# Guenael/rtlsdr-wsprd

Hardware: AMD Instinct MI355X
Metric: 2-minute WSPR segments decoded per second (higher is better)
Workload: dtype f32

## Files before the change

### rtlsdr-wsprd_amd/csrc/kernels/fano_wave.h

```cpp
#pragma once
#include <stdint.h>

#if defined(__HIPCC__)
#define WSPR_FW_HD __host__ __device__ __forceinline__
#else
#define WSPR_FW_HD static inline
#endif

namespace wspr {
namespace fano_wave {

constexpr int kBits = 81, kLast = 80, kTail = 81 - 31, kDelta = 60;
constexpr uint32_t kPolyA = 0xf2d05351u, kPolyB = 0xe4613c47u;
constexpr int kPosDone = 127;

struct Visit { uint32_t st, dlo, meta, gt, led; };

WSPR_FW_HD int      v_pos(const Visit& v)   { return (int)((v.meta >> 18) & 127u); }
WSPR_FW_HD bool     v_retry(const Visit& v) { return (v.meta >> 25) & 1u; }
WSPR_FW_HD int      v_gamma(const Visit& v) { return (int)(int16_t)(v.gt & 0xffffu); }
WSPR_FW_HD int      v_thr(const Visit& v)   { return (int)(int16_t)(v.gt >> 16); }
WSPR_FW_HD uint32_t pack_gt(int g, int t)   { return ((uint32_t)g & 0xffffu) | ((uint32_t)t << 16); }
WSPR_FW_HD uint32_t pack_meta(uint32_t dhi, int pos, bool retry) {
    return (dhi & 0x3ffffu) | ((uint32_t)pos << 18) | ((uint32_t)retry << 25);
}

WSPR_FW_HD unsigned parity32(uint32_t v) {
#if defined(__HIP_DEVICE_COMPILE__)
    return (unsigned)__popc(v) & 1u;
#else
    return (unsigned)__builtin_popcount(v) & 1u;
#endif
}

struct Expansion {
    bool has0, has1, again, done;
    uint32_t look1;
    Visit kid0, kid1, self;
};

WSPR_FW_HD int metric_of(uint32_t lo, uint32_t hi, unsigned pair) {
    const uint32_t w = (pair & 2u) ? hi : lo;
    return (int)(int16_t)((pair & 1u) ? (w >> 16) : (w & 0xffffu));
}

WSPR_FW_HD void expand(const Visit& v, uint32_t bm_lo, uint32_t bm_hi, Expansion& e) {
    const int pos = v_pos(v), g = v_gamma(v), t = v_thr(v);
    const bool tail = pos >= kTail;
    const unsigned zp = (parity32(v.st & kPolyA) << 1) | parity32(v.st & kPolyB);
    const int m0 = metric_of(bm_lo, bm_hi, zp), m1 = metric_of(bm_lo, bm_hi, 3u ^ zp);
    const bool zero_better = tail || (m0 > m1);
    const int best = zero_better ? m0 : m1, second = zero_better ? m1 : m0;
    const uint32_t better = zero_better ? 0u : 1u;
    const int a0 = g + best, a1 = g + second;
    const bool first_visit = g < t + kDelta;
    const bool ok0 = a0 >= t;
    const bool ok1 = ok0 && !tail && a1 >= t;
    e.done = ok0 && pos == kLast;
    e.has0 = ok0 && !e.done;
    e.has1 = ok1;
    e.look1 = (ok0 && !tail) ? 1u : 0u;
    e.again = v_retry(v) && !e.done;
    const bool up0 = first_visit && a0 >= t + kDelta;
    const bool up1 = first_visit && a1 >= t + kDelta;
    uint32_t dlo0 = v.dlo, dhi0 = v.meta & 0x3ffffu, dlo1 = v.dlo, dhi1 = dhi0;
    if (pos < 32)      { dlo0 |= better << pos;        dlo1 |= (better ^ 1u) << pos; }
    else if (pos < 50) { dhi0 |= better << (pos - 32); dhi1 |= (better ^ 1u) << (pos - 32); }
    e.kid0.st = (v.st | better) << 1;
    e.kid0.dlo = dlo0;
    e.kid0.meta = pack_meta(dhi0, pos + 1, up0);
    e.kid0.gt = pack_gt(a0, up0 ? t + kDelta : t);
    e.kid0.led = 0;
    e.kid1.st = (v.st | (better ^ 1u)) << 1;
    e.kid1.dlo = dlo1;
    e.kid1.meta = pack_meta(dhi1, pos + 1, up1);
    e.kid1.gt = pack_gt(a1, up1 ? t + kDelta : t);
    e.kid1.led = 0;
    e.self = v;
    e.self.meta = pack_meta(v.meta & 0x3ffffu, pos, pos == 0);
    e.self.gt = pack_gt(g, t - kDelta);
    e.self.led = 0;
    if (e.done) {
        e.self = v;
        e.self.meta = pack_meta(v.meta & 0x3ffffu, kPosDone, false);
        e.self.gt = pack_gt(a0, t);
    }
}

WSPR_FW_HD void decisions_to_bytes(uint32_t dlo, uint32_t dhi, unsigned char* data10) {
    for (int k = 0; k < 10; ++k) {
        unsigned b = 0;
        for (int j = 0; j < 8; ++j) {
            const int n = 8 * k + j;
            const unsigned bit = n < 32 ? (dlo >> n) & 1u : (n < 50 ? (dhi >> (n - 32)) & 1u : 0u);
            b = (b << 1) | bit;
        }
        data10[k] = (unsigned char)b;
    }
}

struct Result {
    int ret;
    unsigned cycles;
    unsigned metric;
    unsigned steps;
    unsigned char data[10];
};

}
}
```

### rtlsdr-wsprd_amd/csrc/kernels/k6_fano_wave.hip

```cpp
#include "wspr_device.h"
#include "fano_wave.h"
#include <cstdlib>
#include <algorithm>

namespace wspr {
namespace {

using namespace fano_wave;


__device__ __forceinline__ uint32_t wave_scan_add(uint32_t v) {
#define WSPR_DPP(x, ctrl, rmask, bmask) (uint32_t)__builtin_amdgcn_update_dpp(0, (int)(x), ctrl, rmask, bmask, false)
    v += WSPR_DPP(v, 0x111, 0xf, 0xf);
    v += WSPR_DPP(v, 0x112, 0xf, 0xf);
    v += WSPR_DPP(v, 0x114, 0xf, 0xe);
    v += WSPR_DPP(v, 0x118, 0xf, 0xc);
    v += WSPR_DPP(v, 0x142, 0xa, 0xf);
    v += WSPR_DPP(v, 0x143, 0xc, 0xf);
#undef WSPR_DPP
    return v;
}

__device__ __forceinline__ int lanes_below(unsigned long long mask) {
    return (int)__builtin_amdgcn_mbcnt_hi((unsigned)(mask >> 32), __builtin_amdgcn_mbcnt_lo((unsigned)mask, 0u));
}

constexpr int kWin = 512, kHalf = kWin / 2;
static_assert(kHalf >= 64 && kWin - 192 >= kHalf, "a step's pops (<= 64) and pushes (<= 192) must fit beside the half that moves");

template <int kCap>
__global__ __launch_bounds__(64)
void fano_wave_kernel(const unsigned char* __restrict__ symbols, const int* __restrict__ offsets, int n,
                      const short* __restrict__ metric0, unsigned maxcycles,
                      int* __restrict__ ret, unsigned* __restrict__ cycles, unsigned* __restrict__ metric,
                      unsigned* __restrict__ maxnp, unsigned char* __restrict__ data, unsigned* __restrict__ steps_out,
                      uint32_t* __restrict__ gpool, int* __restrict__ next_vector) {
    __shared__ uint32_t lpool[5 * kWin];
    uint32_t* __restrict__ gp = gpool + (size_t)blockIdx.x * 5 * kCap;
    auto ld = [&](int arr, int i) -> uint32_t { return lpool[arr * kWin + (i & (kWin - 1))]; };
    auto st_ = [&](int arr, int i, uint32_t v) { lpool[arr * kWin + (i & (kWin - 1))] = v; };
    auto lds_order = [] {
        __builtin_amdgcn_fence(__ATOMIC_RELEASE, "wavefront");
        __builtin_amdgcn_wave_barrier();
        __builtin_amdgcn_fence(__ATOMIC_ACQUIRE, "wavefront");
    };
    __shared__ uint2 bm[kBits];
    __shared__ unsigned char symd[kNSymD];
    __shared__ short mt[256];
    const int lane = threadIdx.x;
    for (int e = lane; e < 256; e += 64) mt[e] = metric0[e];
    for (;;) {
    int v;
    if (next_vector) {
        int got = 0;
        if (lane == 0) got = atomicAdd(next_vector, 1);
        v = __builtin_amdgcn_readfirstlane(got);
    } else {
        v = blockIdx.x;
    }
    if (v >= n) return;
    __syncthreads();

    {
        const unsigned char* __restrict__ sym = symbols + (size_t)offsets[v] * kNSymD;
        int base = 0;
        for (int c = 0; c < 4; ++c) {
            const int i = 64 * c + lane;
            const int j = (int)(__brev((unsigned)i) >> 24);
            const bool valid = j < kNSymD;
            const unsigned long long m = __ballot(valid);
            if (valid) symd[base + lanes_below(m)] = sym[j];
            base += __popcll(m);
        }
    }
    __syncthreads();
    for (int k = lane; k < kBits; k += 64) {
        const int s0 = symd[2 * k], s1 = symd[2 * k + 1];
        const int a0 = mt[s0], a1 = mt[255 - s0], b0 = mt[s1], b1 = mt[255 - s1];
        bm[k] = make_uint2((uint32_t)(uint16_t)(short)(a0 + b0) | ((uint32_t)(uint16_t)(short)(a0 + b1) << 16),
                           (uint32_t)(uint16_t)(short)(a1 + b0) | ((uint32_t)(uint16_t)(short)(a1 + b1) << 16));
    }
    if (lane == 0) {
        st_(0, 0, 0u); st_(1, 0, 0u); st_(2, 0, pack_meta(0u, 0, true)); st_(3, 0, pack_gt(0, 0)); st_(4, 0, 0u);
    }
    __syncthreads();

    const unsigned budget = maxcycles * (unsigned)kBits;
    int size = 1;
    int lo = 0;
    unsigned settled = 0;
    unsigned steps = 0;
    int rc = -2;
    unsigned out_cycles = 0, out_metric = 0;
    uint32_t out_dlo = 0, out_dhi = 0;

    for (;;) {
        if (settled >= budget) { rc = -1; out_cycles = budget + 2; break; }
        const int room = kCap - size;
        const int wide = size <= kCap / 2 ? 64 : (room > 256 ? 8 : 1);
        const int take = min(min(wide, size), room >> 1);
        if (take < 1 || steps > 4u * budget + 1024u) { rc = -2; break; }
        ++steps;
        if (size - take < lo) {
            __builtin_amdgcn_fence(__ATOMIC_RELEASE, "workgroup");
            __builtin_amdgcn_fence(__ATOMIC_ACQUIRE, "workgroup");
            lo -= kHalf;
#pragma unroll
            for (int arr = 0; arr < 5; ++arr)
#pragma unroll
                for (int u = 0; u < kHalf / 64; ++u) {
                    const int i = lo + 64 * u + lane;
                    lpool[arr * kWin + (i & (kWin - 1))] = gp[arr * kCap + i];
                }
            lds_order();
        }
        const bool active = lane < take;
        const int idx = size - 1 - (active ? lane : 0);
        Visit x{ld(0, idx), ld(1, idx), ld(2, idx), ld(3, idx), ld(4, idx)};
        const int pos = v_pos(x);
        const bool is_done_visit = active && pos == kPosDone;
        if (__builtin_amdgcn_readfirstlane((int)is_done_visit)) {
            const unsigned looks = settled + 1;
            rc = looks >= budget ? -1 : 0;
            out_cycles = looks + 1;
            out_metric = (unsigned)__builtin_amdgcn_readfirstlane(v_gamma(x));
            out_dlo = (uint32_t)__builtin_amdgcn_readfirstlane((int)x.dlo);
            out_dhi = (uint32_t)__builtin_amdgcn_readfirstlane((int)(x.meta & 0x3ffffu));
            break;
        }
        const uint2 q = bm[min(pos, kLast)];
        Expansion e;
        expand(x, q.x, q.y, e);
        const bool stop_here = active && (is_done_visit || e.done);
        const unsigned long long stop_mask = __ballot(stop_here);
        bool live = active;
        int base = size - take;
        if (stop_mask) {
            const int jc = __builtin_ctzll(stop_mask);
            live = active && lane <= jc;
            base = 0;
            lo = 0;
        }
        const bool keep_self = live && (is_done_visit || e.done);
        const bool has0 = live && !keep_self && e.has0;
        const bool has1 = live && !keep_self && e.has1;
        const bool again = live && (keep_self || e.again);
        const int c = (int)has0 + (int)has1 + (int)again;
        if (__ballot(again && !keep_self && v_thr(e.self) < -32000)) { rc = -2; break; }
        const unsigned long long b0 = __ballot(has0), b1 = __ballot(has1), b2 = __ballot(again);
        const int before = lanes_below(b0) + lanes_below(b1) + lanes_below(b2);
        const int total = __popcll(b0) + __popcll(b1) + __popcll(b2);
        const uint32_t back = (live && !keep_self) ? 1u + (c == 0 ? x.led : 0u) : 0u;
        const uint32_t pre = wave_scan_add(back);
        const unsigned long long has_mask = b0 | b1 | b2;
        const unsigned long long later = has_mask & ~((2ull << lane) - 1ull);
        const int nxt = later ? __builtin_ctzll(later) : 63;
        const uint32_t pre_nxt = (uint32_t)__builtin_amdgcn_ds_bpermute(nxt << 2, (int)pre);
        const uint32_t gain = pre_nxt - pre;
        const int first = has_mask ? __builtin_ctzll(has_mask) : 63;
        settled += (uint32_t)__builtin_amdgcn_readlane((int)pre, first);
        if (base + total > lo + kWin) {
#pragma unroll
            for (int arr = 0; arr < 5; ++arr)
#pragma unroll
                for (int u = 0; u < kHalf / 64; ++u) {
                    const int i = lo + 64 * u + lane;
                    gp[arr * kCap + i] = lpool[arr * kWin + (i & (kWin - 1))];
                }
            lo += kHalf;
            lds_order();
        }
        const int top = base + total - 1;
        const uint32_t tail_led = x.led + gain;
        if (has0) {
            const int w = top - before;
            st_(0, w, e.kid0.st); st_(1, w, e.kid0.dlo); st_(2, w, e.kid0.meta); st_(3, w, e.kid0.gt);
            st_(4, w, e.look1 + ((!has1 && !again) ? tail_led : 0u));
        }
        if (has1) {
            const int w = top - before - (int)has0;
            st_(0, w, e.kid1.st); st_(1, w, e.kid1.dlo); st_(2, w, e.kid1.meta); st_(3, w, e.kid1.gt);
            st_(4, w, !again ? tail_led : 0u);
        }
        if (again) {
            const int w = top - before - (int)has0 - (int)has1;
            const Visit s = is_done_visit ? x : e.self;
            st_(0, w, s.st); st_(1, w, s.dlo); st_(2, w, s.meta); st_(3, w, s.gt);
            st_(4, w, keep_self ? 0u : tail_led);
        }
        size = base + total;
        lds_order();
    }
    if (lane == 0) {
        ret[v] = rc;
        cycles[v] = out_cycles;
        if (metric) metric[v] = rc == 0 ? out_metric : 0u;
        if (maxnp) maxnp[v] = rc == 0 ? (unsigned)kLast : 0u;
        unsigned char d[10];
        decisions_to_bytes(out_dlo, out_dhi, d);
        for (int k = 0; k < 10; ++k) data[(size_t)v * 10 + k] = d[k];
        if (steps_out) steps_out[v] = steps;
    }
    if (!next_vector) return;
    }
}

}

#ifndef WSPR_K6W_PER_CU
#define WSPR_K6W_PER_CU 13
#endif
constexpr int kWaveGrid = 256 * WSPR_K6W_PER_CU;

size_t fano_wave_scratch_words(int n) {
    return (size_t)std::min(n, kWaveGrid) * 5 * 4096 + 16;
}

void launch_fano_wave(const unsigned char* symbols, const int* offsets, int n, const short* metric0,
                      unsigned maxcycles, int* ret, unsigned* cycles, unsigned* metric, unsigned* maxnp,
                      unsigned char* data, unsigned* steps, uint32_t* scratch, hipStream_t st) {
    if (n <= 0) return;
    const int grid = std::min(n, kWaveGrid);
    int* counter = reinterpret_cast<int*>(scratch + (size_t)grid * 5 * 4096);
    static const int rep = [] { const char* e = lab_env("WSPR_REPEAT_FANO"); return e ? atoi(e) : 1; }();
    for (int r = 1; r < rep; ++r) {
        (void)hipMemsetAsync(counter, 0, sizeof(int), st);
        hipLaunchKernelGGL((fano_wave_kernel<4096>), dim3(grid), dim3(64), 0, st, symbols, offsets, n, metric0, maxcycles,
                           ret, cycles, metric, maxnp, data, steps, scratch, counter);
    }
    (void)hipMemsetAsync(counter, 0, sizeof(int), st);
    static const bool small = [] { const char* e = lab_env("WSPR_FANO_WAVE_CAP"); return e && atoi(e) == 1024; }();
    if (small)
        hipLaunchKernelGGL((fano_wave_kernel<1024>), dim3(grid), dim3(64), 0, st, symbols, offsets, n, metric0, maxcycles,
                           ret, cycles, metric, maxnp, data, steps, scratch, counter);
    else
        hipLaunchKernelGGL((fano_wave_kernel<4096>), dim3(grid), dim3(64), 0, st, symbols, offsets, n, metric0, maxcycles,
                           ret, cycles, metric, maxnp, data, steps, scratch, counter);
}

}
```

Before: 47220.

## Pack Fano stack entries as uint4, compute lane masks with ballots, add stats variant

Changes the LDS window and global spill pool from five separate 32-bit arrays to a packed uint4 array plus a separate led array. Each stack entry can then be read and written with one 128-bit access instead of four. The per-lane branching for child pushes becomes wave-wide ballot masks with inverse_ballot tests. expand() now uses branchless bit arithmetic for the decision bits and packs meta fields directly. It also adds a compile-time stats mode that reports stack high-water, spill, fill and cut counts through maxnp, plus a 640-capacity variant selected by environment variable. The stats code is compiled out by default, but the larger rewrite may shift register pressure.

```diff
diff --git a/rtlsdr-wsprd_amd/csrc/kernels/fano_wave.h b/rtlsdr-wsprd_amd/csrc/kernels/fano_wave.h
--- a/rtlsdr-wsprd_amd/csrc/kernels/fano_wave.h
+++ b/rtlsdr-wsprd_amd/csrc/kernels/fano_wave.h
@@ -35,13 +35,13 @@
 
 struct Expansion {
     bool has0, has1, again, done;
+    bool ok0, ok1;
     uint32_t look1;
     Visit kid0, kid1, self;
 };
 
 WSPR_FW_HD int metric_of(uint32_t lo, uint32_t hi, unsigned pair) {
-    const uint32_t w = (pair & 2u) ? hi : lo;
-    return (int)(int16_t)((pair & 1u) ? (w >> 16) : (w & 0xffffu));
+    return (int)(int16_t)(uint16_t)((((uint64_t)hi << 32) | lo) >> ((16u * pair) & 63u));
 }
 
 WSPR_FW_HD void expand(const Visit& v, uint32_t bm_lo, uint32_t bm_hi, Expansion& e) {
@@ -56,6 +56,8 @@
     const bool first_visit = g < t + kDelta;
     const bool ok0 = a0 >= t;
     const bool ok1 = ok0 && !tail && a1 >= t;
+    e.ok0 = ok0;
+    e.ok1 = a1 >= t;
     e.done = ok0 && pos == kLast;
     e.has0 = ok0 && !e.done;
     e.has1 = ok1;
@@ -63,21 +65,23 @@
     e.again = v_retry(v) && !e.done;
     const bool up0 = first_visit && a0 >= t + kDelta;
     const bool up1 = first_visit && a1 >= t + kDelta;
-    uint32_t dlo0 = v.dlo, dhi0 = v.meta & 0x3ffffu, dlo1 = v.dlo, dhi1 = dhi0;
-    if (pos < 32)      { dlo0 |= better << pos;        dlo1 |= (better ^ 1u) << pos; }
-    else if (pos < 50) { dhi0 |= better << (pos - 32); dhi1 |= (better ^ 1u) << (pos - 32); }
+    const uint64_t bit = (uint64_t)(pos < kTail ? 1u : 0u) << (pos & 63);
+    const uint32_t blo = (uint32_t)bit, bhi = (uint32_t)(bit >> 32);
+    const uint32_t dlo0 = v.dlo | (better ? blo : 0u), dlo1 = dlo0 ^ blo;
+    const uint32_t kmeta = (v.meta & 0x1ffffffu) + (1u << 18);
+    const uint32_t meta0 = kmeta | (better ? bhi : 0u), meta1 = meta0 ^ bhi;
     e.kid0.st = (v.st | better) << 1;
     e.kid0.dlo = dlo0;
-    e.kid0.meta = pack_meta(dhi0, pos + 1, up0);
+    e.kid0.meta = meta0 | ((uint32_t)up0 << 25);
     e.kid0.gt = pack_gt(a0, up0 ? t + kDelta : t);
     e.kid0.led = 0;
     e.kid1.st = (v.st | (better ^ 1u)) << 1;
     e.kid1.dlo = dlo1;
-    e.kid1.meta = pack_meta(dhi1, pos + 1, up1);
+    e.kid1.meta = meta1 | ((uint32_t)up1 << 25);
     e.kid1.gt = pack_gt(a1, up1 ? t + kDelta : t);
     e.kid1.led = 0;
     e.self = v;
-    e.self.meta = pack_meta(v.meta & 0x3ffffu, pos, pos == 0);
+    e.self.meta = (v.meta & 0x1ffffffu) | ((uint32_t)(pos == 0) << 25);
     e.self.gt = pack_gt(g, t - kDelta);
     e.self.led = 0;
     if (e.done) {
diff --git a/rtlsdr-wsprd_amd/csrc/kernels/k6_fano_wave.hip b/rtlsdr-wsprd_amd/csrc/kernels/k6_fano_wave.hip
--- a/rtlsdr-wsprd_amd/csrc/kernels/k6_fano_wave.hip
+++ b/rtlsdr-wsprd_amd/csrc/kernels/k6_fano_wave.hip
@@ -21,24 +21,28 @@
     return v;
 }
 
-__device__ __forceinline__ int lanes_below(unsigned long long mask) {
-    return (int)__builtin_amdgcn_mbcnt_hi((unsigned)(mask >> 32), __builtin_amdgcn_mbcnt_lo((unsigned)mask, 0u));
-}
+using mask64 = unsigned long long;
+
+__device__ __forceinline__ int lanes_below(mask64 mask, int add = 0) {
+    return (int)__builtin_amdgcn_mbcnt_hi((unsigned)(mask >> 32), __builtin_amdgcn_mbcnt_lo((unsigned)mask, (unsigned)add));
+}
+__device__ __forceinline__ mask64 lanes_where(bool p) { return __builtin_amdgcn_ballot_w64(p); }
+__device__ __forceinline__ bool in_mask(mask64 m) { return __builtin_amdgcn_inverse_ballot_w64(m); }
 
 constexpr int kWin = 512, kHalf = kWin / 2;
 static_assert(kHalf >= 64 && kWin - 192 >= kHalf, "a step's pops (<= 64) and pushes (<= 192) must fit beside the half that moves");
 
-template <int kCap>
+template <int kCap, bool kStats>
 __global__ __launch_bounds__(64)
 void fano_wave_kernel(const unsigned char* __restrict__ symbols, const int* __restrict__ offsets, int n,
                       const short* __restrict__ metric0, unsigned maxcycles,
                       int* __restrict__ ret, unsigned* __restrict__ cycles, unsigned* __restrict__ metric,
                       unsigned* __restrict__ maxnp, unsigned char* __restrict__ data, unsigned* __restrict__ steps_out,
                       uint32_t* __restrict__ gpool, int* __restrict__ next_vector) {
-    __shared__ uint32_t lpool[5 * kWin];
-    uint32_t* __restrict__ gp = gpool + (size_t)blockIdx.x * 5 * kCap;
-    auto ld = [&](int arr, int i) -> uint32_t { return lpool[arr * kWin + (i & (kWin - 1))]; };
-    auto st_ = [&](int arr, int i, uint32_t v) { lpool[arr * kWin + (i & (kWin - 1))] = v; };
+    __shared__ uint4 win[kWin];
+    __shared__ uint32_t wled[kWin];
+    uint4* __restrict__ gp4 = reinterpret_cast<uint4*>(gpool + (size_t)blockIdx.x * 5 * kCap);
+    uint32_t* __restrict__ gpl = gpool + (size_t)blockIdx.x * 5 * kCap + 4 * kCap;
     auto lds_order = [] {
         __builtin_amdgcn_fence(__ATOMIC_RELEASE, "wavefront");
         __builtin_amdgcn_wave_barrier();
@@ -48,6 +52,7 @@
     __shared__ unsigned char symd[kNSymD];
     __shared__ short mt[256];
     const int lane = threadIdx.x;
+    const mask64 after_me = ~((2ull << lane) - 1ull) | (1ull << 63);
     for (int e = lane; e < 256; e += 64) mt[e] = metric0[e];
     for (;;) {
     int v;
@@ -68,7 +73,7 @@
             const int i = 64 * c + lane;
             const int j = (int)(__brev((unsigned)i) >> 24);
             const bool valid = j < kNSymD;
-            const unsigned long long m = __ballot(valid);
+            const mask64 m = lanes_where(valid);
             if (valid) symd[base + lanes_below(m)] = sym[j];
             base += __popcll(m);
         }
@@ -81,7 +86,8 @@
                            (uint32_t)(uint16_t)(short)(a1 + b0) | ((uint32_t)(uint16_t)(short)(a1 + b1) << 16));
     }
     if (lane == 0) {
-        st_(0, 0, 0u); st_(1, 0, 0u); st_(2, 0, pack_meta(0u, 0, true)); st_(3, 0, pack_gt(0, 0)); st_(4, 0, 0u);
+        win[0] = make_uint4(0u, 0u, pack_meta(0u, 0, true), pack_gt(0, 0));
+        wled[0] = 0u;
     }
     __syncthreads();
 
@@ -93,12 +99,15 @@
     int rc = -2;
     unsigned out_cycles = 0, out_metric = 0;
     uint32_t out_dlo = 0, out_dhi = 0;
+    int st_size = 1, st_spills = 0, st_fills = 0, st_cuts = 0;
 
     for (;;) {
         if (settled >= budget) { rc = -1; out_cycles = budget + 2; break; }
         const int room = kCap - size;
         const int wide = size <= kCap / 2 ? 64 : (room > 256 ? 8 : 1);
-        const int take = min(min(wide, size), room >> 1);
+        int take = min(wide, size);
+        asm volatile("" : "+s"(take));
+        take = min(take, room >> 1);
         if (take < 1 || steps > 4u * budget + 1024u) { rc = -2; break; }
         ++steps;
         if (size - take < lo) {
@@ -106,20 +115,21 @@
             __builtin_amdgcn_fence(__ATOMIC_ACQUIRE, "workgroup");
             lo -= kHalf;
 #pragma unroll
-            for (int arr = 0; arr < 5; ++arr)
-#pragma unroll
-                for (int u = 0; u < kHalf / 64; ++u) {
-                    const int i = lo + 64 * u + lane;
-                    lpool[arr * kWin + (i & (kWin - 1))] = gp[arr * kCap + i];
-                }
+            for (int u = 0; u < kHalf / 64; ++u) {
+                const int i = lo + 64 * u + lane;
+                win[i & (kWin - 1)] = gp4[i];
+                wled[i & (kWin - 1)] = gpl[i];
+            }
+            if (kStats) ++st_fills;
             lds_order();
         }
-        const bool active = lane < take;
-        const int idx = size - 1 - (active ? lane : 0);
-        Visit x{ld(0, idx), ld(1, idx), ld(2, idx), ld(3, idx), ld(4, idx)};
+        const mask64 active_m = take >= 64 ? ~0ull : (1ull << take) - 1ull;
+        const int slot = (size - 1 - lane) & (kWin - 1);
+        const uint4 xw = win[slot];
+        Visit x{xw.x, xw.y, xw.z, xw.w, wled[slot]};
         const int pos = v_pos(x);
-        const bool is_done_visit = active && pos == kPosDone;
-        if (__builtin_amdgcn_readfirstlane((int)is_done_visit)) {
+        const mask64 donev_m = lanes_where(pos == kPosDone) & active_m;
+        if (donev_m & 1ull) {
             const unsigned looks = settled + 1;
             rc = looks >= budget ? -1 : 0;
             out_cycles = looks + 1;
@@ -131,71 +141,74 @@
         const uint2 q = bm[min(pos, kLast)];
         Expansion e;
         expand(x, q.x, q.y, e);
-        const bool stop_here = active && (is_done_visit || e.done);
-        const unsigned long long stop_mask = __ballot(stop_here);
-        bool live = active;
+        const mask64 ok0_m = lanes_where(e.ok0), tail_m = lanes_where(pos >= kTail);
+        const mask64 done_m = ok0_m & lanes_where(pos == kLast);
+        const mask64 has0_m = ok0_m & ~done_m;
+        const mask64 has1_m = ok0_m & lanes_where(e.ok1) & ~tail_m;
+        const mask64 again_m = lanes_where((x.meta & (1u << 25)) != 0u) & ~done_m;
+        const mask64 stop_m = (donev_m | done_m) & active_m;
+        mask64 live_m = active_m;
         int base = size - take;
-        if (stop_mask) {
-            const int jc = __builtin_ctzll(stop_mask);
-            live = active && lane <= jc;
+        if (stop_m) {
+            live_m = active_m & (stop_m ^ (stop_m - 1ull));
             base = 0;
+            if (kStats && lo > 0) ++st_cuts;
             lo = 0;
         }
-        const bool keep_self = live && (is_done_visit || e.done);
-        const bool has0 = live && !keep_self && e.has0;
-        const bool has1 = live && !keep_self && e.has1;
-        const bool again = live && (keep_self || e.again);
-        const int c = (int)has0 + (int)has1 + (int)again;
-        if (__ballot(again && !keep_self && v_thr(e.self) < -32000)) { rc = -2; break; }
-        const unsigned long long b0 = __ballot(has0), b1 = __ballot(has1), b2 = __ballot(again);
-        const int before = lanes_below(b0) + lanes_below(b1) + lanes_below(b2);
-        const int total = __popcll(b0) + __popcll(b1) + __popcll(b2);
-        const uint32_t back = (live && !keep_self) ? 1u + (c == 0 ? x.led : 0u) : 0u;
+        const mask64 keep_m = live_m & stop_m;
+        const mask64 open_m = live_m & ~keep_m;
+        const mask64 s0_m = has0_m & open_m, s1_m = has1_m & open_m;
+        const mask64 s2_m = keep_m | (again_m & open_m);
+        if ((s2_m & ~keep_m) & lanes_where(v_thr(e.self) < -32000)) { rc = -2; break; }
+        const mask64 has_m = s0_m | s1_m | s2_m;
+        const int before = lanes_below(s0_m, lanes_below(s1_m, lanes_below(s2_m)));
+        const int total = __popcll(s0_m) + __popcll(s1_m) + __popcll(s2_m);
+        const uint32_t back = in_mask(open_m) ? (in_mask(has_m) ? 1u : 1u + x.led) : 0u;
         const uint32_t pre = wave_scan_add(back);
-        const unsigned long long has_mask = b0 | b1 | b2;
-        const unsigned long long later = has_mask & ~((2ull << lane) - 1ull);
-        const int nxt = later ? __builtin_ctzll(later) : 63;
+        const int nxt = __builtin_ctzll((has_m | (1ull << 63)) & after_me);
         const uint32_t pre_nxt = (uint32_t)__builtin_amdgcn_ds_bpermute(nxt << 2, (int)pre);
         const uint32_t gain = pre_nxt - pre;
-        const int first = has_mask ? __builtin_ctzll(has_mask) : 63;
+        const int first = has_m ? __builtin_ctzll(has_m) : 63;
         settled += (uint32_t)__builtin_amdgcn_readlane((int)pre, first);
         if (base + total > lo + kWin) {
 #pragma unroll
-            for (int arr = 0; arr < 5; ++arr)
-#pragma unroll
-                for (int u = 0; u < kHalf / 64; ++u) {
-                    const int i = lo + 64 * u + lane;
-                    gp[arr * kCap + i] = lpool[arr * kWin + (i & (kWin - 1))];
-                }
+            for (int u = 0; u < kHalf / 64; ++u) {
+                const int i = lo + 64 * u + lane;
+                gp4[i] = win[i & (kWin - 1)];
+                gpl[i] = wled[i & (kWin - 1)];
+            }
             lo += kHalf;
+            if (kStats) ++st_spills;
             lds_order();
         }
-        const int top = base + total - 1;
         const uint32_t tail_led = x.led + gain;
-        if (has0) {
-            const int w = top - before;
-            st_(0, w, e.kid0.st); st_(1, w, e.kid0.dlo); st_(2, w, e.kid0.meta); st_(3, w, e.kid0.gt);
-            st_(4, w, e.look1 + ((!has1 && !again) ? tail_led : 0u));
-        }
-        if (has1) {
-            const int w = top - before - (int)has0;
-            st_(0, w, e.kid1.st); st_(1, w, e.kid1.dlo); st_(2, w, e.kid1.meta); st_(3, w, e.kid1.gt);
-            st_(4, w, !again ? tail_led : 0u);
-        }
-        if (again) {
-            const int w = top - before - (int)has0 - (int)has1;
-            const Visit s = is_done_visit ? x : e.self;
-            st_(0, w, s.st); st_(1, w, s.dlo); st_(2, w, s.meta); st_(3, w, s.gt);
-            st_(4, w, keep_self ? 0u : tail_led);
+        int w = base + total - 1 - before;
+        if (in_mask(s0_m)) {
+            win[w & (kWin - 1)] = make_uint4(e.kid0.st, e.kid0.dlo, e.kid0.meta, e.kid0.gt);
+            wled[w & (kWin - 1)] = e.look1 + (in_mask(s1_m | s2_m) ? 0u : tail_led);
+        }
+        w -= (int)in_mask(s0_m);
+        if (in_mask(s1_m)) {
+            win[w & (kWin - 1)] = make_uint4(e.kid1.st, e.kid1.dlo, e.kid1.meta, e.kid1.gt);
+            wled[w & (kWin - 1)] = in_mask(s2_m) ? 0u : tail_led;
+        }
+        w -= (int)in_mask(s1_m);
+        if (in_mask(s2_m)) {
+            const Visit s = in_mask(donev_m) ? x : e.self;
+            win[w & (kWin - 1)] = make_uint4(s.st, s.dlo, s.meta, s.gt);
+            wled[w & (kWin - 1)] = in_mask(keep_m) ? 0u : tail_led;
         }
         size = base + total;
+        if (kStats) st_size = max(st_size, size);
         lds_order();
     }
     if (lane == 0) {
         ret[v] = rc;
         cycles[v] = out_cycles;
         if (metric) metric[v] = rc == 0 ? out_metric : 0u;
-        if (maxnp) maxnp[v] = rc == 0 ? (unsigned)kLast : 0u;
+        if (maxnp) maxnp[v] = kStats ? (unsigned)st_size | ((unsigned)min(st_spills, 63) << 13) | ((unsigned)min(st_fills, 63) << 19) |
+                                           ((unsigned)min(st_cuts, 63) << 25)
+                                     : (rc == 0 ? (unsigned)kLast : 0u);
         unsigned char d[10];
         decisions_to_bytes(out_dlo, out_dhi, d);
         for (int k = 0; k < 10; ++k) data[(size_t)v * 10 + k] = d[k];
@@ -222,20 +235,21 @@
     if (n <= 0) return;
     const int grid = std::min(n, kWaveGrid);
     int* counter = reinterpret_cast<int*>(scratch + (size_t)grid * 5 * 4096);
+    auto launch = [&](auto kernel) {
+        (void)hipMemsetAsync(counter, 0, sizeof(int), st);
+        hipLaunchKernelGGL(kernel, dim3(grid), dim3(64), 0, st, symbols, offsets, n, metric0, maxcycles,
+                           ret, cycles, metric, maxnp, data, steps, scratch, counter);
+    };
     static const int rep = [] { const char* e = lab_env("WSPR_REPEAT_FANO"); return e ? atoi(e) : 1; }();
-    for (int r = 1; r < rep; ++r) {
-        (void)hipMemsetAsync(counter, 0, sizeof(int), st);
-        hipLaunchKernelGGL((fano_wave_kernel<4096>), dim3(grid), dim3(64), 0, st, symbols, offsets, n, metric0, maxcycles,
-                           ret, cycles, metric, maxnp, data, steps, scratch, counter);
-    }
-    (void)hipMemsetAsync(counter, 0, sizeof(int), st);
-    static const bool small = [] { const char* e = lab_env("WSPR_FANO_WAVE_CAP"); return e && atoi(e) == 1024; }();
-    if (small)
-        hipLaunchKernelGGL((fano_wave_kernel<1024>), dim3(grid), dim3(64), 0, st, symbols, offsets, n, metric0, maxcycles,
-                           ret, cycles, metric, maxnp, data, steps, scratch, counter);
-    else
-        hipLaunchKernelGGL((fano_wave_kernel<4096>), dim3(grid), dim3(64), 0, st, symbols, offsets, n, metric0, maxcycles,
-                           ret, cycles, metric, maxnp, data, steps, scratch, counter);
-}
-
-}
+    for (int r = 1; r < rep; ++r) launch(fano_wave_kernel<4096, false>);
+    const char* cap_env = lab_env("WSPR_FANO_WAVE_CAP");
+    const char* stats_env = lab_env("WSPR_FANO_WAVE_STATS");
+    const int cap = cap_env ? atoi(cap_env) : 4096;
+    const bool report = stats_env && atoi(stats_env) == 1;
+    if (cap == 1024) { if (report) launch(fano_wave_kernel<1024, true>); else launch(fano_wave_kernel<1024, false>); }
+    else if (cap == 640) { if (report) launch(fano_wave_kernel<640, true>); else launch(fano_wave_kernel<640, false>); }
+    else if (report) launch(fano_wave_kernel<4096, true>);
+    else launch(fano_wave_kernel<4096, false>);
+}
+
+}
```

Result: no change. 47770 (median of 2 runs) (+1.2%).
